# Rengar-Yang/humanoid-gym-with-comments

Measured on AMD Instinct MI355X. Metric: env-steps/sec (whole node) at 4096 envs + PPO iters/sec, 1/2/4/8 MI355X, higher is better.
Workload: dtype f32; 1 GPU; XBot-L flat terrain, 4096 envs/GPU, PPO 24-step rollout (BASELINE configs[1]); envs_per_gpu=4096, num_steps_per_env=24, parallelism=dp1, ppo=2 epochs x 4 minibatches, actor 705-512-256-128-12, critic 219-768-256-128-1, update_graph=one, gemm_table=tuning/tunableop_mi355x_f32.csv

## Files before the change

### humanoid-gym-with-comments_amd/csrc/hg_gemm.hip

```cpp
#include <hip/hip_runtime.h>
#include <stdint.h>

#include <type_traits>

#include "hg_common.h"

namespace {

typedef float f32x16 __attribute__((ext_vector_type(16)));
typedef float f32x4u __attribute__((ext_vector_type(4), aligned(4)));

struct GemmArgs {
  const float* A;
  int64_t lda;
  const float* B;
  int64_t ldb;
  const float* bias;
  const float* Y;
  int64_t ldY;
  float* C;
  int64_t ldc;
  float* colpart;
  int64_t M;
  int N, K;
// ... 906 lines not shown
  __device__ __forceinline__ void load(const float* __restrict__ P, int64_t ld, int64_t r0, int64_t rend, int col0,
                                       int ncols, int tid) {
#pragma unroll
    for (int j = 0; j < IPT; j++) {
      const int idx = tid + j * NT;
      if (ITEMS % NT != 0 && idx >= ITEMS) break;
      const int row = idx / (COLS / 4), c = col0 + 4 * (idx % (COLS / 4));
      const int64_t r = r0 + row;
      const float* p = P + r * ld + c;
      if (r < rend && c + 3 < ncols) {
        const f32x4u x = *reinterpret_cast<const f32x4u*>(p);
        v[j][0] = x[0]; v[j][1] = x[1]; v[j][2] = x[2]; v[j][3] = x[3];
      } else {
#pragma unroll
        for (int e = 0; e < 4; e++) v[j][e] = (r < rend && c + e < ncols) ? p[e] : 0.f;
      }
    }
  }
  __device__ __forceinline__ void store(char* __restrict__ S, int tid) const {
#pragma unroll
    for (int j = 0; j < IPT; j++) {
      const int idx = tid + j * NT;
      if (ITEMS % NT != 0 && idx >= ITEMS) break;
      const int row = idx / (COLS / 4), c4 = idx % (COLS / 4);
      uint2 x0, x1, x2;
      split3x4(v[j], x0, x1, x2);
      char* d = S + row * PITCH + 8 * c4;
      *reinterpret_cast<uint2*>(d) = x0;
      *reinterpret_cast<uint2*>(d + PLANE) = x1;
      *reinterpret_cast<uint2*>(d + 2 * PLANE) = x2;
    }
  }
};

template <int PITCH>
__device__ __forceinline__ bf16x8 tr_operand(const char* __restrict__ plane, int c0, int lane) {
  const int g = lane >> 4, q = (lane >> 2) & 3, p = lane & 3;
  const char* a = plane + (8 * (g >> 1) + q) * PITCH + 2 * (c0 + 16 * (g & 1) + 4 * p);
  typedef __attribute__((address_space(3))) s16x4 lds_s16x4;
  const s16x4 lo = __builtin_amdgcn_ds_read_tr16_b64_v4i16((lds_s16x4*)(a));
  const s16x4 hi = __builtin_amdgcn_ds_read_tr16_b64_v4i16((lds_s16x4*)(a + 4 * PITCH));
  const short e[8] = {lo[0], lo[1], lo[2], lo[3], hi[0], hi[1], hi[2], hi[3]};
  return __builtin_bit_cast(bf16x8, e);
}

template <int WGM, int WGN, int TM, int TN, int PF>
__global__ void __launch_bounds__(64 * WGM * WGN) k_wgrad_tr(WgradArgs w) {
  constexpr int NT = 64 * WGM * WGN;
  constexpr int BM = 32 * TM * WGM, BN = 32 * TN * WGN;
  typedef TrStage<BM, NT> SA;
  typedef TrStage<BN, NT> SB;
  constexpr int STAGE = 3 * SA::PLANE + 3 * SB::PLANE;
  __shared__ __attribute__((aligned(16))) char lds[2 * STAGE];
  const int tid = threadIdx.x, lane = tid & 63, wave = tid >> 6;
  const int i = lane & 31, h = lane >> 5;
  const unsigned nb = gridDim.x;
  unsigned L = blockIdx.x;
  if ((nb & 7u) == 0) L = (blockIdx.x & 7u) * (nb >> 3) + (blockIdx.x >> 3);
  if ((int64_t)L >= w.tiles * w.slices) return;
  const int slice = (int)((int64_t)L / w.tiles);
  const int64_t tile = (int64_t)L % w.tiles;
  const int m0 = (int)(tile / w.tiles_n) * BM, n0 = (int)(tile % w.tiles_n) * BN;
  const int wm0 = (wave % WGM) * (32 * TM), wn0 = (wave / WGM) * (32 * TN);
  const int64_t kbeg = (int64_t)slice * w.kslice;
  const int64_t kend = min<int64_t>(w.R, kbeg + w.kslice);
  const int nchunks = kend > kbeg ? (int)((kend - kbeg + 15) / 16) : 0;

  f32x16 acc[TM][TN];
#pragma unroll
  for (int m = 0; m < TM; m++)
#pragma unroll
    for (int n = 0; n < TN; n++) acc[m][n] = (f32x16)0.f;

  auto step = [&](int c, SA& la, SB& lb, const SA& ha, const SB& hb) {
    const char* cur = lds + (c & 1) * STAGE;
    char* nxt = lds + ((c + 1) & 1) * STAGE;
    if (c + PF < nchunks) {
      const int64_t r0 = kbeg + (int64_t)(c + PF) * 16;
      la.load(w.A, w.lda, r0, kend, m0, w.M, tid);
      lb.load(w.B, w.ldb, r0, kend, n0, w.N, tid);
    }
    bf16x8 a[3][TM], b[3][TN];
#pragma unroll
    for (int p = 0; p < 3; p++) {
#pragma unroll
      for (int m = 0; m < TM; m++) a[p][m] = tr_operand<SA::PITCH>(cur + p * SA::PLANE, wm0 + 32 * m, lane);
#pragma unroll
      for (int n = 0; n < TN; n++)
        b[p][n] = tr_operand<SB::PITCH>(cur + 3 * SA::PLANE + p * SB::PLANE, wn0 + 32 * n, lane);
    }
#pragma unroll
    for (int m = 0; m < TM; m++)
#pragma unroll
      for (int n = 0; n < TN; n++) {
        acc[m][n] = __builtin_amdgcn_mfma_f32_32x32x16_bf16(a[2][m], b[0][n], acc[m][n], 0, 0, 0);
        acc[m][n] = __builtin_amdgcn_mfma_f32_32x32x16_bf16(a[1][m], b[1][n], acc[m][n], 0, 0, 0);
        acc[m][n] = __builtin_amdgcn_mfma_f32_32x32x16_bf16(a[0][m], b[2][n], acc[m][n], 0, 0, 0);
        acc[m][n] = __builtin_amdgcn_mfma_f32_32x32x16_bf16(a[1][m], b[0][n], acc[m][n], 0, 0, 0);
        acc[m][n] = __builtin_amdgcn_mfma_f32_32x32x16_bf16(a[0][m], b[1][n], acc[m][n], 0, 0, 0);
        acc[m][n] = __builtin_amdgcn_mfma_f32_32x32x16_bf16(a[0][m], b[0][n], acc[m][n], 0, 0, 0);
      }
    if (c + 1 < nchunks) {
      ha.store(nxt, tid);
      hb.store(nxt + 3 * SA::PLANE, tid);
    }
    __syncthreads();
  };
  SA sa0, sa1;
  SB sb0, sb1;
  if (nchunks > 0) {
    sa0.load(w.A, w.lda, kbeg, kend, m0, w.M, tid);
    sb0.load(w.B, w.ldb, kbeg, kend, n0, w.N, tid);
    sa0.store(lds, tid);
    sb0.store(lds + 3 * SA::PLANE, tid);
    if (PF == 2 && nchunks > 1) {
      sa1.load(w.A, w.lda, kbeg + 16, kend, m0, w.M, tid);
      sb1.load(w.B, w.ldb, kbeg + 16, kend, n0, w.N, tid);
    }
  }
  __syncthreads();
  if (PF == 1) {
    for (int c = 0; c < nchunks; c++) step(c, sa0, sb0, sa0, sb0);
  } else {
    for (int c = 0; c < nchunks; c += 2) {
      step(c, sa0, sb0, sa1, sb1);
      if (c + 1 < nchunks) step(c + 1, sa1, sb1, sa0, sb0);
    }
  }
  float* Cs = w.C + (int64_t)slice * w.cstride;
#pragma unroll
  for (int n = 0; n < TN; n++) {
    const int col = n0 + wn0 + 32 * n + i;
    if (col >= w.N) continue;
#pragma unroll
    for (int m = 0; m < TM; m++)
#pragma unroll
      for (int q = 0; q < 16; q++) {
        const int row = m0 + wm0 + 32 * m + (q & 3) + 8 * (q >> 2) + 4 * h;
        if (row < w.M) Cs[(int64_t)row * w.ldc + col] = acc[m][n][q];
      }
  }
}

template <int WGM, int WGN, int TM, int TN, int PF = 1>
int launch_wgrad_tr(WgradArgs w, hipStream_t s) {
  constexpr int BM = 32 * TM * WGM, BN = 32 * TN * WGN;
  w.tiles_n = (w.N + BN - 1) / BN;
  w.tiles = (int64_t)((w.M + BM - 1) / BM) * w.tiles_n;
  if (w.tiles * w.slices > 0x7fffffff) return HG_ERR_ARG;
  hipLaunchKernelGGL((k_wgrad_tr<WGM, WGN, TM, TN, PF>), dim3((unsigned)(w.tiles * w.slices)), dim3(64 * WGM * WGN), 0, s, w);
  return hipGetLastError() == hipSuccess ? HG_OK : HG_ERR_HIP;
}

constexpr int WGRAD_TR0 = 40, WGRAD_TR1 = 54;

}

extern "C" int64_t hg_gemm_x6_image_bytes(int64_t rows, int64_t K) {
  if (rows <= 0 || K <= 0 || rows > 0x7fffffff || K > 0x7fffffff) return -1;
  return img_chunks(K) * 3 * img_rows(rows) * 2 * 16;
}

extern "C" int hg_gemm_x6_image_jobs_pitched(const float* const* P, const int64_t* ld, const int* trans,
                                             const int64_t* rows, const int64_t* K, void* const* img,
                                             const int64_t* pitch_rows, int njobs, void* stream);

extern "C" int hg_gemm_x6_image_jobs(const float* const* P, const int64_t* ld, const int* trans, const int64_t* rows,
                                     const int64_t* K, void* const* img, int njobs, void* stream) {
  return hg_gemm_x6_image_jobs_pitched(P, ld, trans, rows, K, img, nullptr, njobs, stream);
}

extern "C" int hg_gemm_x6_image_jobs_pitched(const float* const* P, const int64_t* ld, const int* trans,
                                             const int64_t* rows, const int64_t* K, void* const* img,
                                             const int64_t* pitch_rows, int njobs, void* stream) {
  if (njobs <= 0) return HG_OK;
  if (njobs > IMG_MAX || !P || !ld || !trans || !rows || !K || !img) return HG_ERR_ARG;
  ImageJobs J;
  J.njobs = njobs;
  int64_t blocks = 0;
  for (int j = 0; j < njobs; j++) {
    if (!P[j] || !img[j] || rows[j] <= 0 || K[j] <= 0 || rows[j] > 0x7fffffff || K[j] > 0x7fffffff ||
        (trans[j] != 0 && trans[j] != 1))
      return HG_ERR_ARG;
    if ((trans[j] == 0 && ld[j] < K[j]) || (trans[j] == 1 && ld[j] < rows[j])) return HG_ERR_ARG;
    if ((uintptr_t)P[j] % 4 || (uintptr_t)img[j] % 16) return HG_ERR_ARG;
    J.P[j] = P[j];
    J.img[j] = reinterpret_cast<bf16x8*>(img[j]);
    J.ld[j] = ld[j];
    const int64_t prow = pitch_rows && pitch_rows[j] > 0 ? pitch_rows[j] : rows[j];
    if (prow < rows[j] || prow > 0x7fffffff) return HG_ERR_ARG;
    J.pitch[j] = img_rows(prow) * 2;
    J.trans[j] = trans[j];
    J.R[j] = (int)rows[j];
    J.K[j] = (int)K[j];
    J.groups[j] = (int)(img_rows(rows[j]) / 128);
    J.block0[j] = (int)blocks;
    blocks += img_chunks(K[j]) * J.groups[j];
    if (blocks > (int64_t)1 << 30) return HG_ERR_ARG;
  }
  J.block0[njobs] = (int)blocks;
  for (int j = 0; j < njobs;) {
    const int64_t prow = pitch_rows && pitch_rows[j] > 0 ? pitch_rows[j] : rows[j];
    int64_t sum = rows[j];
    int e = j + 1;
    while (e < njobs && pitch_rows && pitch_rows[e] == prow && K[e] == K[j] && sum < prow &&
           (uintptr_t)img[e] == (uintptr_t)img[e - 1] + (uintptr_t)(32 * rows[e - 1])) {
      sum += rows[e];
      e++;
    }
    if (sum != prow) return HG_ERR_ARG;
    for (int b = j; b + 1 < e; b++)
      if (rows[b] % 256) return HG_ERR_ARG;
    j = e;
  }
  hipLaunchKernelGGL(k_x6_image_jobs, dim3((unsigned)blocks), dim3(256), 0, (hipStream_t)stream, J);
  return hipGetLastError() == hipSuccess ? HG_OK : HG_ERR_HIP;
}

extern "C" int hg_gemm_f32_img(int mode, const float* A, int64_t lda, const void* Aimg, const void* Bimg,
                               const float* bias, const float* Y, int64_t ldY, float* C, int64_t ldc, float* colpart,
                               int64_t M, int N, int K, int act, int tile, int64_t aimg_bytes, int64_t bimg_bytes,
                               void* stream) {
  if ((!A && !Aimg) || !Bimg || !C || M <= 0 || N <= 0 || K <= 0 || ldc < N || (mode != 0 && mode != 1) || act < 0 ||
      act > 1 || tile < 19 || tile > NTILES_IMG)
    return HG_ERR_ARG;
  if (!Aimg && lda < K) return HG_ERR_ARG;
  if (bimg_bytes != hg_gemm_x6_image_bytes(N, K) || (Aimg && aimg_bytes != hg_gemm_x6_image_bytes(M, K)))
    return HG_ERR_ARG;
  if (mode == 1 && act == 1 && (!Y || ldY < N)) return HG_ERR_ARG;
  if ((!Aimg && (uintptr_t)A % 4) || (uintptr_t)Aimg % 16 || (uintptr_t)Bimg % 16 || (uintptr_t)C % 4)
    return HG_ERR_ARG;
  const bool vec = !Aimg && lda % 4 == 0 && (uintptr_t)A % 16 == 0;
  const float* a = Aimg ? reinterpret_cast<const float*>(Aimg) : A;
  const int64_t la = Aimg ? img_rows(M) * 2 : lda;
  GemmArgs g{a, la, reinterpret_cast<const float*>(Bimg), img_rows(N) * 2, bias, Y, ldY, C, ldc, colpart, M, N, K, 0, 0};
  GemmX6Args xa{g, 0, 0, 1};
  return x6_img_dispatch(tile, mode, Aimg ? 3 : 1, xa, vec, act == 1, (hipStream_t)stream);
}

extern "C" int hg_gemm_f32_img_split(const float* A, int64_t lda, const void* Bimg, const float* bias,
                                     const float* bias2, float* C, int64_t ldc, float* C2, int64_t ldc2, int nsplit,
                                     int64_t M, int N, int K, int act, int tile, int64_t bimg_bytes, void* stream) {
  if (!A || !Bimg || !C || !C2 || !bias != !bias2 || M <= 0 || N <= 0 || K <= 0 || nsplit <= 0 || nsplit >= N || nsplit % 256 ||
      ldc < nsplit || ldc2 < N - nsplit || lda < K || act < 0 || act > 1 || tile < 19 || tile > NTILES_IMG)
    return HG_ERR_ARG;
  if (bimg_bytes != hg_gemm_x6_image_bytes(N, K)) return HG_ERR_ARG;
  if ((uintptr_t)A % 4 || (uintptr_t)Bimg % 16 || (uintptr_t)C % 4 || (uintptr_t)C2 % 4) return HG_ERR_ARG;
  const bool vec = lda % 4 == 0 && (uintptr_t)A % 16 == 0;
  GemmArgs g{A, lda, reinterpret_cast<const float*>(Bimg), img_rows(N) * 2, bias, nullptr, 0, C, ldc, nullptr, M, N, K,
             0, 0, C2, ldc2, nsplit, bias2};
  GemmX6Args xa{g, 0, 0, 1};
  return x6_img_dispatch(tile, 0, 1, xa, vec, act == 1, (hipStream_t)stream);
}

extern "C" int hg_gemm_wgrad_img(const void* Aimg, const void* Bimg, float* C, int64_t ldc, int64_t cstride, int64_t M,
                                 int N, int64_t K, int slices, int tile, int64_t aimg_bytes, int64_t bimg_bytes,
                                 void* stream) {
  if (!Aimg || !Bimg || !C || M <= 0 || N <= 0 || K <= 0 || K > 0x7fffffff || ldc < N || slices < 1 || tile < 19 ||
      tile > NTILES)
    return HG_ERR_ARG;
  if (aimg_bytes != hg_gemm_x6_image_bytes(M, K) || bimg_bytes != hg_gemm_x6_image_bytes(N, K)) return HG_ERR_ARG;
  if (slices > 1 && cstride < M * (int64_t)ldc) return HG_ERR_ARG;
  if ((uintptr_t)Aimg % 16 || (uintptr_t)Bimg % 16 || (uintptr_t)C % 4) return HG_ERR_ARG;
  GemmArgs g{reinterpret_cast<const float*>(Aimg), img_rows(M) * 2, reinterpret_cast<const float*>(Bimg),
             img_rows(N) * 2, nullptr, nullptr, 0, C, ldc, nullptr, M, N, (int)K, 0, 0};
  const int64_t kslice = ((K + slices - 1) / slices + 31) & ~(int64_t)31;
  GemmX6Args xa{g, kslice, cstride, slices};
  return x6_img_dispatch(tile, 2, 3, xa, false, false, (hipStream_t)stream);
}

extern "C" int hg_gemm_tile(int mode, int64_t M, int N, int K) {
  (void)mode;
  (void)K;
  const int64_t t16 = ((M + 127) / 128) * ((N + 63) / 64);
  return t16 >= 768 ? 16 : 5;
}

extern "C" int64_t hg_gemm_colpart_rows(int64_t M, int tile) {
  if (tile < 1 || tile > NTILES_IMG) return -1;
  const int bm = tile_bm(tile);
  return (M + bm - 1) / bm;
}

extern "C" int hg_gemm_f32(int mode, const float* A, int64_t lda, const float* B, int64_t ldb, const float* bias,
                           const float* Y, int64_t ldY, float* C, int64_t ldc, float* colpart, int64_t M, int N, int K,
                           int act, int tile, void* stream) {
  if (tile == 30) tile = 25;
  else if (tile == 31) tile = 22;
  else if (tile == 32) tile = 21;
  if (!A || !B || !C || M <= 0 || N <= 0 || K <= 0 || lda < K || ldc < N || mode < 0 || mode > 3 || mode == 2 ||
      act < 0 || act > 1 || tile < 1 || tile > NTILES)
    return HG_ERR_ARG;
  if (mode == 3 && tile < 19) return HG_ERR_ARG;
  if ((mode == 0 || mode == 3) && ldb < K) return HG_ERR_ARG;
  if (mode == 1 && ldb < N) return HG_ERR_ARG;
  if ((mode == 1 || mode == 3) && act == 1 && (!Y || ldY < N)) return HG_ERR_ARG;
  if ((uintptr_t)A % 4 || (uintptr_t)B % 4 || (uintptr_t)C % 4) return HG_ERR_ARG;
  const bool vec = lda % 4 == 0 && (uintptr_t)A % 16 == 0 &&
                   (mode == 1 || (ldb % 4 == 0 && (uintptr_t)B % 16 == 0));
  GemmArgs g{A, lda, B, ldb, bias, Y, ldY, C, ldc, colpart, M, N, K, 0, 0};
  hipStream_t s = (hipStream_t)stream;
  const bool elu = act == 1;
  switch (tile) {
    case 1: return launch<128, 128, 2, 2, 32, 0>(mode, g, vec, elu, s);
    case 2: return launch<128, 64, 2, 2, 32, 0>(mode, g, vec, elu, s);
    case 3: return launch<64, 128, 2, 2, 32, 0>(mode, g, vec, elu, s);
    case 4: return launch<64, 64, 2, 2, 32, 0>(mode, g, vec, elu, s);
    case 5: return launch<64, 64, 2, 2, 32, 1>(mode, g, vec, elu, s);
    case 6: return launch<64, 64, 2, 2, 64, 0>(mode, g, vec, elu, s);
    case 7: return launch<64, 64, 2, 2, 64, 1>(mode, g, vec, elu, s);
    case 8: return launch<128, 64, 4, 2, 32, 1>(mode, g, vec, elu, s);
    case 9: return launch<128, 128, 2, 4, 32, 1>(mode, g, vec, elu, s);
    case 10: return launch<128, 64, 2, 2, 64, 1>(mode, g, vec, elu, s);
    case 11: return launch<64, 64, 2, 2, 16, 1>(mode, g, vec, elu, s);
    case 12: return launch<128, 128, 2, 4, 16, 1>(mode, g, vec, elu, s);
    case 13: return launch<128, 64, 4, 2, 16, 1>(mode, g, vec, elu, s);
    case 14: return launch<64, 128, 2, 2, 16, 1>(mode, g, vec, elu, s);
    case 15: return launch<64, 64, 2, 2, 32, 1, 1>(mode, g, vec, elu, s);
    case 16: return launch<128, 64, 4, 2, 32, 1, 1>(mode, g, vec, elu, s);
    case 17: return launch<128, 128, 2, 4, 32, 1, 1>(mode, g, vec, elu, s);
    case 18: return launch<64, 64, 2, 2, 16, 1, 1>(mode, g, vec, elu, s);
    default: break;
  }
  GemmX6Args xa{g, 0, 0, 1};
  switch (tile) {
    case 20: return launch_x6<128, 128, 2, 2, 1>(mode, xa, vec, elu, s);
    case 21: return launch_x6<128, 128, 2, 4, 1>(mode, xa, vec, elu, s);
    case 22: return launch_x6<128, 64, 2, 2, 1>(mode, xa, vec, elu, s);
    case 29:
    case 23: return launch_x6<64, 64, 2, 2, 1>(mode, xa, vec, elu, s);
    case 24: return launch_x6<128, 128, 2, 2, 2>(mode, xa, vec, elu, s);
    case 25: return launch_x6<256, 128, 4, 2, 1>(mode, xa, vec, elu, s);
    case 26: return launch_x6<128, 128, 2, 4, 2>(mode, xa, vec, elu, s);
    case 27: return launch_x6<128, 256, 2, 4, 1>(mode, xa, vec, elu, s);
    case 28: return launch_x6<64, 256, 2, 4, 1>(mode, xa, vec, elu, s);
    default: return launch_x6<64, 128, 2, 2, 1>(mode, xa, vec, elu, s);
  }
}

extern "C" int hg_gemm_f32_wgrad(const float* A, int64_t lda, const float* B, int64_t ldb, float* C, int64_t ldc,
                                 int64_t cstride, int64_t M, int N, int64_t K, int slices, int kmajor, int tile,
                                 void* stream) {
  const bool tr = tile >= WGRAD_TR0 && tile <= WGRAD_TR1;
  if (!A || !B || !C || M <= 0 || N <= 0 || K <= 0 || ldc < N || slices < 1 || (!tr && (tile < 19 || tile > 28)) ||
      K > 0x7fffffff || (kmajor != 0 && kmajor != 1) || (tr && (kmajor != 0 || M > 0x7fffffff)))
    return HG_ERR_ARG;
  if (kmajor == 0 && (lda < M || ldb < N)) return HG_ERR_ARG;
  if (kmajor == 1 && (lda < K || ldb < K)) return HG_ERR_ARG;
  if (slices > 1 && cstride < M * (int64_t)ldc) return HG_ERR_ARG;
  if ((uintptr_t)A % 4 || (uintptr_t)B % 4 || (uintptr_t)C % 4) return HG_ERR_ARG;
  const int64_t kslice = ((K + slices - 1) / slices + 15) & ~(int64_t)15;
  hipStream_t s = (hipStream_t)stream;
  if (tr) {
    WgradArgs w{A, lda, B, ldb, C, ldc, cstride, (int)M, N, K, kslice, slices, 0, 0};
    switch (tile) {
      case 40: return launch_wgrad_tr<4, 2, 2, 3>(w, s);
      case 41: return launch_wgrad_tr<4, 2, 2, 2>(w, s);
      case 42: return launch_wgrad_tr<2, 2, 2, 2>(w, s);
      case 43: return launch_wgrad_tr<2, 4, 2, 2>(w, s);
      case 44: return launch_wgrad_tr<2, 2, 2, 3>(w, s);
      case 45: return launch_wgrad_tr<4, 2, 1, 2>(w, s);
      case 46: return launch_wgrad_tr<2, 2, 1, 1>(w, s);
      case 47: return launch_wgrad_tr<2, 2, 1, 2>(w, s);
      case 48: return launch_wgrad_tr<2, 2, 2, 1>(w, s);
      case 49: return launch_wgrad_tr<4, 2, 2, 3, 2>(w, s);
      case 50: return launch_wgrad_tr<4, 2, 2, 2, 2>(w, s);
      case 51: return launch_wgrad_tr<2, 2, 2, 2, 2>(w, s);
      case 52: return launch_wgrad_tr<2, 2, 1, 1, 2>(w, s);
      case 53: return launch_wgrad_tr<2, 2, 1, 2, 2>(w, s);
      default: return launch_wgrad_tr<4, 2, 1, 2, 2>(w, s);
    }
  }
  GemmArgs g{A, lda, B, ldb, nullptr, nullptr, 0, C, ldc, nullptr, M, N, (int)K, 0, 0};
  GemmX6Args xa{g, kslice, cstride, slices};
  const int md = kmajor ? 4 : 2;
  const bool vec = kmajor && lda % 4 == 0 && ldb % 4 == 0 && (uintptr_t)A % 16 == 0 && (uintptr_t)B % 16 == 0;
  switch (tile) {
    case 20: return launch_x6<128, 128, 2, 2, 1>(md, xa, vec, false, s);
    case 21: return launch_x6<128, 128, 2, 4, 1>(md, xa, vec, false, s);
    case 22: return launch_x6<128, 64, 2, 2, 1>(md, xa, vec, false, s);
    case 23: return launch_x6<64, 64, 2, 2, 1>(md, xa, vec, false, s);
    case 24: return launch_x6<128, 128, 2, 2, 2>(md, xa, vec, false, s);
    case 25: return launch_x6<256, 128, 4, 2, 1>(md, xa, vec, false, s);
    case 26: return launch_x6<128, 128, 2, 4, 2>(md, xa, vec, false, s);
    case 27: return launch_x6<128, 256, 2, 4, 1>(md, xa, vec, false, s);
    case 28: return launch_x6<64, 256, 2, 4, 1>(md, xa, vec, false, s);
    default: return launch_x6<64, 128, 2, 2, 1>(md, xa, vec, false, s);
  }
}

namespace {
template <bool ELU, int SC>
__global__ void __launch_bounds__(256) k_splitk_finish(const float* __restrict__ ws, int64_t sstride,
                                                       const float* __restrict__ bias, float* __restrict__ C,
                                                       int64_t ldc, int64_t M, int N, int S, bool vec) {
  const int nq = (N + 3) >> 2;
  const int64_t t = (int64_t)blockIdx.x * 256 + threadIdx.x;
  if (t >= M * nq) return;
  const int64_t m = t / nq;
  const int n0 = (int)(t % nq) * 4;
  const float* p = ws + m * N + n0;
  float v[4];
  if (vec) {
    float4 a;
    if (SC > 0) {
      typedef float fin4 __attribute__((ext_vector_type(4)));
      fin4 x[SC > 0 ? SC : 1];
#pragma unroll
      for (int s = 0; s < SC; s++) x[s] = __builtin_nontemporal_load(reinterpret_cast<const fin4*>(p + s * sstride));
#pragma unroll
      for (int s = 1; s < SC; s++) { x[0].x += x[s].x; x[0].y += x[s].y; x[0].z += x[s].z; x[0].w += x[s].w; }
      a = make_float4(x[0].x, x[0].y, x[0].z, x[0].w);
    } else {
      a = *reinterpret_cast<const float4*>(p);
      for (int s = 1; s < S; s++) {
        const float4 b = *reinterpret_cast<const float4*>(p + s * sstride);
        a.x += b.x; a.y += b.y; a.z += b.z; a.w += b.w;
      }
    }
    const float4 bb = *reinterpret_cast<const float4*>(bias + n0);
    v[0] = a.x + bb.x; v[1] = a.y + bb.y; v[2] = a.z + bb.z; v[3] = a.w + bb.w;
#pragma unroll
    for (int q = 0; q < 4; q++)
      if (ELU) v[q] = v[q] > 0.f ? v[q] : expm1f(v[q]);
    *reinterpret_cast<float4*>(C + m * ldc + n0) = make_float4(v[0], v[1], v[2], v[3]);
  } else {
    for (int q = 0; q < 4 && n0 + q < N; q++) {
      float a = p[q];
      for (int s = 1; s < S; s++) a += p[q + s * sstride];
      float x = a + bias[n0 + q];
      if (ELU) x = x > 0.f ? x : expm1f(x);
      C[m * ldc + n0 + q] = x;
    }
  }
}

int splitk_finish(const float* ws, const float* bias, float* C, int64_t ldc, int64_t M, int N, int slices, bool elu,
                  hipStream_t s) {
  const int64_t threads = M * ((N + 3) / 4);
  const bool fvec = N % 4 == 0 && ldc % 4 == 0 && (uintptr_t)C % 16 == 0 && (uintptr_t)bias % 16 == 0;
  const dim3 grid((unsigned)((threads + 255) / 256)), block(256);
#define HG_FIN(E, SC) hipLaunchKernelGGL((k_splitk_finish<E, SC>), grid, block, 0, s, ws, M * (int64_t)N, bias, C, ldc, M, N, \
                                         slices, fvec)
  if (elu) {
    if (slices == 4) HG_FIN(true, 4);
    else if (slices == 2) HG_FIN(true, 2);
    else HG_FIN(true, 0);
  } else {
    if (slices == 4) HG_FIN(false, 4);
    else if (slices == 2) HG_FIN(false, 2);
    else HG_FIN(false, 0);
  }
#undef HG_FIN
  return hipGetLastError() == hipSuccess ? HG_OK : HG_ERR_HIP;
}
}

extern "C" int64_t hg_gemm_splitk_kslice(int K, int slices) {
  if (K <= 0 || slices < 1) return -1;
  return (((int64_t)K + slices - 1) / slices + 15) & ~(int64_t)15;
}

extern "C" int hg_gemm_f32_splitk(const float* A, int64_t lda, const float* B, int64_t ldb, const float* bias,
                                  float* C, int64_t ldc, float* ws, int64_t ws_floats, int64_t M, int N, int K,
                                  int act, int tile, int slices, void* stream) {
  if (!A || !B || !bias || !C || !ws || M <= 0 || N <= 0 || K <= 0 || lda < K || ldb < K || ldc < N ||
      act < 0 || act > 1 || tile < 20 || tile > 28 || slices < 2 || slices > 16)
    return HG_ERR_ARG;
  const int64_t kslice = hg_gemm_splitk_kslice(K, slices);
  if ((slices - 1) * kslice >= K) return HG_ERR_ARG;
  if (ws_floats < slices * M * (int64_t)N) return HG_ERR_ARG;
  if ((uintptr_t)A % 4 || (uintptr_t)B % 4 || (uintptr_t)C % 4 || (uintptr_t)bias % 4 || (uintptr_t)ws % 16)
    return HG_ERR_ARG;
  const int64_t threads = M * ((N + 3) / 4);
  if ((threads + 255) / 256 > 0x7fffffff) return HG_ERR_ARG;
  hipStream_t s = (hipStream_t)stream;
  GemmArgs g{A, lda, B, ldb, nullptr, nullptr, 0, ws, N, nullptr, M, N, K, 0, 0};
  GemmX6Args xa{g, kslice, M * (int64_t)N, slices};
  const bool vec = lda % 4 == 0 && ldb % 4 == 0 && (uintptr_t)A % 16 == 0 && (uintptr_t)B % 16 == 0;
  const bool elu = act == 1;
  const int md = 4;
  int rc;
  switch (tile) {
    case 20: rc = launch_x6<128, 128, 2, 2, 1>(md, xa, vec, elu, s); break;
    case 21: rc = launch_x6<128, 128, 2, 4, 1>(md, xa, vec, elu, s); break;
    case 22: rc = launch_x6<128, 64, 2, 2, 1>(md, xa, vec, elu, s); break;
    case 23: rc = launch_x6<64, 64, 2, 2, 1>(md, xa, vec, elu, s); break;
    case 24: rc = launch_x6<128, 128, 2, 2, 2>(md, xa, vec, elu, s); break;
    case 25: rc = launch_x6<256, 128, 4, 2, 1>(md, xa, vec, elu, s); break;
    case 26: rc = launch_x6<128, 128, 2, 4, 2>(md, xa, vec, elu, s); break;
    case 27: rc = launch_x6<128, 256, 2, 4, 1>(md, xa, vec, elu, s); break;
    default: rc = launch_x6<64, 256, 2, 4, 1>(md, xa, vec, elu, s); break;
  }
  if (rc != HG_OK) return rc;
  return splitk_finish(ws, bias, C, ldc, M, N, slices, elu, s);
}

extern "C" int hg_gemm_f32_splitk_img(const float* A, int64_t lda, const void* Bimg, int64_t bimg_bytes,
                                      const float* bias, float* C, int64_t ldc, float* ws, int64_t ws_floats,
                                      int64_t M, int N, int K, int act, int tile, int slices, void* stream) {
  if (!A || !Bimg || !bias || !C || !ws || M <= 0 || N <= 0 || K <= 0 || lda < K || ldc < N || act < 0 || act > 1 ||
      tile < 19 || tile > NTILES_IMG || tile == 24 || tile == 26 || tile == 29 || slices < 2 || slices > 16)
    return HG_ERR_ARG;
  if (bimg_bytes != hg_gemm_x6_image_bytes(N, K)) return HG_ERR_ARG;
  const int64_t kslice = hg_gemm_splitk_kslice(K, slices);
  if ((slices - 1) * kslice >= K) return HG_ERR_ARG;
  if (ws_floats < slices * M * (int64_t)N) return HG_ERR_ARG;
  if ((uintptr_t)A % 4 || (uintptr_t)Bimg % 16 || (uintptr_t)C % 4 || (uintptr_t)bias % 4 || (uintptr_t)ws % 16)
    return HG_ERR_ARG;
  if ((M * ((N + 3) / 4) + 255) / 256 > 0x7fffffff) return HG_ERR_ARG;
  hipStream_t s = (hipStream_t)stream;
  GemmArgs g{A, lda, reinterpret_cast<const float*>(Bimg), img_rows(N) * 2, nullptr, nullptr, 0, ws, N, nullptr, M, N,
             K, 0, 0};
  GemmX6Args xa{g, kslice, M * (int64_t)N, slices};
  const bool vec = lda % 4 == 0 && (uintptr_t)A % 16 == 0;
  const int rc = x6_img_dispatch(tile, 4, 1, xa, vec, false, s);
  if (rc != HG_OK) return rc;
  return splitk_finish(ws, bias, C, ldc, M, N, slices, act == 1, s);
}
```

### humanoid-gym-with-comments_amd/humanoid/algo/ppo/hg_mlp.py

```python
import contextlib
import ctypes
import os

import torch
import torch.nn as nn
import torch.nn.functional as F

from humanoid import _native as N


def fusable(net):
    mods = list(net)
    if not mods or not isinstance(mods[-1], nn.Linear):
        return False
    for i, m in enumerate(mods):
        want = nn.Linear if i % 2 == 0 else nn.ELU
        if not isinstance(m, want):
            return False
        if isinstance(m, nn.ELU) and (m.alpha != 1.0 or m.inplace):
            return False
        if isinstance(m, nn.Linear) and m.bias is None:
            return False
    return True


class _Reductions:

    def __init__(self):
        self.jobs = []

    def add(self, src, dst, width, parts):
        self.jobs.append((src, dst, int(width), int(parts)))

    def launch(self, dev):
        n = len(self.jobs)
        if n == 0:
            return
        vp = ctypes.c_void_p
        src = (vp * n)(*[j[0].data_ptr() for j in self.jobs])
        dst = (vp * n)(*[j[1].data_ptr() for j in self.jobs])
        width = (ctypes.c_int64 * n)(*[j[2] for j in self.jobs])
        parts = (ctypes.c_int * n)(*[j[3] for j in self.jobs])
        rc = N.lib().hg_colsum_jobs(src, dst, width, parts, n, _stream(dev))
        if rc != 0:
            raise RuntimeError(f"hg_colsum_jobs failed ({rc})")
        self.jobs = []


def _act_backward(gy, y, rows, width, gb, red=None):
    L = N.lib()
    scratch = torch.empty(int(L.hg_mlp_act_backward_scratch(rows, width)), dtype=torch.float32, device=gy.device)
    gh = torch.empty_like(gy) if y is not None else gy
    s = ctypes.c_void_p(torch.cuda.current_stream(gy.device).cuda_stream)
    rc = L.hg_mlp_act_backward(gy.data_ptr(), y.data_ptr() if y is not None else None,
                               gh.data_ptr() if y is not None else None, rows, width,
                               gb.data_ptr() if red is None else None, scratch.data_ptr(), s)
    if rc != 0:
        raise RuntimeError(f"hg_mlp_act_backward failed ({rc})")
    if red is not None:
        red.add(scratch, gb, width, scratch.numel() // width)
    return gh


def _stream(dev):
    return ctypes.c_void_p(torch.cuda.current_stream(dev).cuda_stream)


def _skinny_ok(h, W):
    n, k = W.shape
    return (bool(N.lib().hg_linear_skinny_supported(n, k)) and h.dim() == 2 and h.stride(1) == 1
            and h.stride(0) % 4 == 0 and h.data_ptr() % 16 == 0 and W.is_contiguous())


def _skinny_forward(h, W, b, out=None):
    rows, n = h.shape[0], W.shape[0]
    y = torch.empty(rows, n, dtype=torch.float32, device=h.device) if out is None else out
    if y.numel() != rows * n or not y.is_contiguous() or y.dtype != torch.float32:
        raise RuntimeError("skinny forward: out must be a contiguous float32 tensor of rows x n elements")
    rc = N.lib().hg_linear_skinny_forward(h.data_ptr(), h.stride(0), W.data_ptr(), b.data_ptr(), y.data_ptr(), rows,
                                          n, W.shape[1], _stream(h.device))
    if rc != 0:
        raise RuntimeError(f"hg_linear_skinny_forward failed ({rc})")
    return y


def _skinny_backward(g, h, W, need_dx, red=None):
    rows, (n, k) = g.shape[0], W.shape
    L = N.lib()
    wb = torch.empty(n * k + n, dtype=torch.float32, device=g.device)
    dx = torch.empty(rows, k, dtype=torch.float32, device=g.device) if need_dx else None
    scratch = torch.empty(int(L.hg_linear_skinny_backward_scratch(rows, n, k)), dtype=torch.float32, device=g.device)
    rc = L.hg_linear_skinny_backward(g.data_ptr(), h.data_ptr(), h.stride(0), W.data_ptr(),
                                     dx.data_ptr() if need_dx else None, wb.data_ptr() if red is None else None,
                                     rows, n, k, scratch.data_ptr(), _stream(g.device))
    if rc != 0:
        raise RuntimeError(f"hg_linear_skinny_backward failed ({rc})")
    if red is not None:
        red.add(scratch, wb, n * k + n, scratch.numel() // (n * k + n))
    return wb[: n * k].view(n, k), wb[n * k:], dx


def _skinny_backward_act(g, h, W, red):
    rows, (n, k) = g.shape[0], W.shape
    L = N.lib()
    wb = torch.empty(n * k + n, dtype=torch.float32, device=g.device)
    gh_prev = torch.empty(rows, k, dtype=torch.float32, device=g.device)
    parts = int(L.hg_linear_skinny_colpart_rows(rows))
    cp = torch.empty(parts, k, dtype=torch.float32, device=g.device)
    gb_prev = torch.empty(k, dtype=torch.float32, device=g.device)
    scratch = torch.empty(int(L.hg_linear_skinny_backward_scratch(rows, n, k)), dtype=torch.float32, device=g.device)
    rc = L.hg_linear_skinny_backward_act(g.data_ptr(), h.data_ptr(), h.stride(0), W.data_ptr(), gh_prev.data_ptr(),
                                         cp.data_ptr(), rows, n, k, scratch.data_ptr(), _stream(g.device))
    if rc != 0:
        raise RuntimeError(f"hg_linear_skinny_backward_act failed ({rc})")
    r = red if red is not None else _Reductions()
    r.add(scratch, wb, n * k + n, scratch.numel() // (n * k + n))
    r.add(cp, gb_prev, k, parts)
    if red is None:
        r.launch(g.device)
    return wb[: n * k].view(n, k), wb[n * k:], gh_prev, gb_prev


_BIG_ROWS = 1 << 40
_DW_SPLIT = {(128, 256): 32, (128, 128): 16, (256, 512): 4, (128, 705): 8, (512, 705): 16, (768, 219): 32,
             (256, 768): 4}


WGRAD_TR = os.environ.get("HG_WGRAD_TR", "1") != "0"
_GEMM_DW = {(512, 705): [(8191, 0), (_BIG_ROWS, (49, 32))],
            (256, 768): [(8191, 0), (_BIG_ROWS, (49, 64))]} if WGRAD_TR else {}
if WGRAD_TR:
    _GEMM_DW[(768, 780)] = [(8191, 0), (_BIG_ROWS, (49, 32))]
_GEMM_DW_EXTRA = {(256, 512): (54, 64), (768, 219): (54, 64), (128, 705): (48, 64), (128, 256): (54, 128),
                  (128, 128): (46, 128)}
_sel = os.environ.get("HG_WGRAD_TR", "1")
if _sel not in ("0", "1"):
    for _shape, _route_tr in _GEMM_DW_EXTRA.items():
        if _sel == "all" or "%dx%d" % _shape in _sel.split(","):
            _GEMM_DW[_shape] = [(8191, 0), (_BIG_ROWS, _route_tr)]


def _weight_grad(gh, x, red=None):
    rows, n = gh.shape
    k = x.shape[1]
    ok = red is not None and gh.is_contiguous() and x.dim() == 2 and x.stride(1) == 1
    route = _route(_GEMM_DW, rows, n, k) if ok else 0
    if route:
        tile, S = route
        L = N.lib()
        part = torch.empty(S, n, k, dtype=torch.float32, device=gh.device)
        rc = L.hg_gemm_f32_wgrad(gh.data_ptr(), gh.stride(0), x.data_ptr(), x.stride(0), part.data_ptr(), k, n * k,
                                 n, k, rows, S, 0, tile, _stream(gh.device))
        if rc != 0:
            raise RuntimeError(f"hg_gemm_f32_wgrad failed ({rc})")
        dw = torch.empty(n, k, dtype=torch.float32, device=gh.device)
        red.add(part, dw, n * k, S)
        return dw
    S = _DW_SPLIT.get((n, k), 1) if rows >= 8192 else 1
    if S == 1 or rows % S or not (gh.is_contiguous() and x.is_contiguous()):
        return torch.mm(gh.t(), x)
    chunks = torch.bmm(gh.view(S, rows // S, n).transpose(1, 2), x.view(S, rows // S, k))
    if red is None:
        return chunks.sum(0)
    dw = torch.empty(n, k, dtype=torch.float32, device=gh.device)
    red.add(chunks, dw, n * k, S)
    return dw


_FUSED_FWD_ROWS = {(512, 256): 8192, (256, 128): 8192, (128, 128): 32768}
FUSED_FORWARD = os.environ.get("HG_FUSED_FORWARD", "1") != "0"


def _fused_ok(h, W, b):
    rows = h.shape[0]
    k = W.shape[1]
    return (FUSED_FORWARD and rows <= _FUSED_FWD_ROWS.get((k, W.shape[0]), 0) and h.dim() == 2 and h.stride(1) == 1
            and h.dtype == torch.float32 and W.is_contiguous() and b is not None and b.is_contiguous())


def linear_act(h, W, b, elu=True, out=None, tile=0):
    rows, n = h.shape[0], W.shape[0]
    y = torch.empty(rows, n, dtype=torch.float32, device=h.device) if out is None else out
    if y.shape != (rows, n) or y.stride(1) != 1 or y.dtype != torch.float32:
        raise RuntimeError("linear_act: out must be a float32 [rows, n] tensor with unit column stride")
    rc = N.lib().hg_linear_act_forward(h.data_ptr(), h.stride(0), W.data_ptr(), b.data_ptr(), y.data_ptr(),
                                       y.stride(0), rows, n, W.shape[1], 1 if elu else 0, tile, _stream(h.device))
    if rc != 0:
        raise RuntimeError(f"hg_linear_act_forward failed ({rc})")
    return y


_BIG = 1 << 40
X6_TILE0 = 19
_GEMM_FWD = {(705, 512): [(8192, 5), (_BIG, 20)], (512, 256): [(8192, 5), (_BIG, 22)],
             (256, 128): [(8192, 0), (32768, 5), (_BIG, 20)], (705, 128): [(8192, 5), (_BIG, 29)],
             (128, 128): [(8192, 0), (_BIG, 5)], (219, 768): [(8192, 21), (_BIG, 32)],
             (768, 256): [(32768, 22), (_BIG, 20)]}
if os.environ.get("HG_X6_APF", "1") == "0":
    _GEMM_FWD[(705, 128)] = [(8192, 5), (_BIG, 23)]
_GEMM_FWD[(780, 768)] = _GEMM_FWD[(219, 768)]
_GEMM_DX = {(256, 512): [(_BIG, 22)], (128, 256): [(_BIG, 31)], (256, 768): [(_BIG, 31)], (128, 128): [(_BIG, 5)]}
GEMM = os.environ.get("HG_GEMM", "1") != "0"
X6_IMAGE = os.environ.get("HG_X6_IMAGE", "1") != "0"
SKINNY_ACT = os.environ.get("HG_SKINNY_ACT", "1") != "0"


def _route(table, rows, k, n):
    if not GEMM:
        return 0
    for max_rows, tile in table.get((k, n), ()):
        if rows <= max_rows:
            return tile
    return 0


def _gemm_fwd_tile(h, W, b):
    if not (h.dim() == 2 and h.stride(1) == 1 and h.dtype == torch.float32 and W.is_contiguous() and b is not None
            and b.is_contiguous()):
        return 0
    return _route(_GEMM_FWD, h.shape[0], W.shape[1], W.shape[0])


_GEMM_FWD_SPLITK = {(705, 512): [(4096, (25, 4))]}
SPLITK_FWD = os.environ.get("HG_SPLITK_FWD", "1") != "0"
if os.environ.get("HG_SPLITK_ROUTE"):
    _GEMM_FWD_SPLITK[(705, 512)] = [(4096, tuple(int(v) for v in os.environ["HG_SPLITK_ROUTE"].split(",")))]


def _gemm_fwd_splitk(h, W, b):
    if not SPLITK_FWD or not _gemm_fwd_tile(h, W, b):
        return None
    for max_rows, route in _GEMM_FWD_SPLITK.get((W.shape[1], W.shape[0]), ()):
        if h.shape[0] <= max_rows:
            return route
    return None


def gemm_forward_splitk(h, W, b, tile, slices, elu=True):
    rows, n, k = h.shape[0], W.shape[0], W.shape[1]
    y = torch.empty(rows, n, dtype=torch.float32, device=h.device)
    ws = torch.empty(slices * rows * n, dtype=torch.float32, device=h.device)
    rc = N.lib().hg_gemm_f32_splitk(h.data_ptr(), h.stride(0), W.data_ptr(), W.stride(0), b.data_ptr(), y.data_ptr(),
                                    y.stride(0), ws.data_ptr(), ws.numel(), rows, n, k, 1 if elu else 0, tile, slices,
                                    _stream(h.device))
    if rc != 0:
        raise RuntimeError(f"hg_gemm_f32_splitk failed ({rc})")
    return y


def _img_rows(r):
    return (r + 255) // 256 * 256


def x6_images(jobs, dev):
    if not jobs:
        return []
    L = N.lib()

    def rows_of(j):
        return sum(P.shape[0] for P in j[1]) if j[0] == "stack" else j[2]

    sizes = [int(L.hg_gemm_x6_image_bytes(rows_of(j), j[-1])) for j in jobs]
    buf = torch.empty(sum(sizes) // 4, dtype=torch.float32, device=dev)
    imgs, off = [], 0
    for sz in sizes:
        imgs.append(buf[off // 4:(off + sz) // 4])
        off += sz
    cj = []
    for j, im in zip(jobs, imgs):
        if j[0] == "stack":
            total, r0 = rows_of(j), 0
            for P in j[1]:
                if r0 % 256:
                    raise ValueError("x6_images: stacked bands must start on a multiple of 256 rows "
                                     "(every band but the last a multiple of 256 rows)")
                cj.append((P, 0, P.shape[0], j[2], im.data_ptr() + 32 * r0, total))
                r0 += P.shape[0]
        else:
            cj.append((j[0], j[1], j[2], j[3], im.data_ptr(), 0))
    m = len(cj)
    vp = ctypes.c_void_p
    i64 = ctypes.c_int64
    rc = L.hg_gemm_x6_image_jobs_pitched((vp * m)(*[c[0].data_ptr() for c in cj]), (i64 * m)(*[c[0].stride(0) for c in cj]),
                                         (ctypes.c_int * m)(*[c[1] for c in cj]), (i64 * m)(*[c[2] for c in cj]),
                                         (i64 * m)(*[c[3] for c in cj]), (vp * m)(*[c[4] for c in cj]),
                                         (i64 * m)(*[c[5] for c in cj]), m, _stream(dev))
    if rc != 0:
        raise RuntimeError(f"hg_gemm_x6_image_jobs_pitched failed ({rc})")
    return imgs
# ... 533 lines not shown
```

Measured before the change: 5.885 million env-steps/s.

## Add software-pipelined transposed wgrad kernel with interleaved staging and MFMA scheduling

Adds a new weight-gradient kernel variant (tile 56) that double-buffers LDS stages and prefetches two chunks ahead in registers. It interleaves the bf16x3 split stores of the next stage between MFMA groups using sched_group_barrier, and adds an edge path that shifts partial-tile loads instead of masking them. It becomes the default route for the large 512x705, 256x768 and 768x780 wgrad shapes in place of tile 49. The goal is to hide global-load and LDS-staging latency behind the matrix math, at the cost of higher register pressure and more complex scheduling.

```diff
diff --git a/humanoid-gym-with-comments_amd/csrc/hg_gemm.hip b/humanoid-gym-with-comments_amd/csrc/hg_gemm.hip
--- a/humanoid-gym-with-comments_amd/csrc/hg_gemm.hip
+++ b/humanoid-gym-with-comments_amd/csrc/hg_gemm.hip
@@ -1082,7 +1082,337 @@
   return hipGetLastError() == hipSuccess ? HG_OK : HG_ERR_HIP;
 }
 
-constexpr int WGRAD_TR0 = 40, WGRAD_TR1 = 54;
+template <int COLS, int NT, int W>
+struct TrStageP {
+  static constexpr int CG = COLS / W;
+  static constexpr int TPR = NT / 16;
+  static_assert(NT % 16 == 0 && CG % TPR == 0 && (W == 2 || W == 4), "every thread carries CG / TPR items of its row");
+  static constexpr int IPT = CG / TPR;
+  static constexpr int PITCH = COLS * 2 + 64;
+  static constexpr int PLANE = 16 * PITCH;
+  typedef float vecu __attribute__((ext_vector_type(W), aligned(4)));
+  struct Map {
+    uint32_t goff;
+    int lds;
+    __device__ __forceinline__ void init(int64_t ld, int col0, int tid) {
+      const int row = tid / TPR, cg = tid % TPR;
+      goff = (uint32_t)(((int64_t)row * ld + col0 + W * cg) * 4);
+      lds = row * PITCH + 2 * W * cg;
+    }
+  };
+  struct EdgeMap {
+    uint32_t goff[IPT];
+    bool on[IPT][3];
+    __device__ __forceinline__ void init(int64_t ld, int col0, int ncols, int tid) {
+      const int row = tid / TPR;
+#pragma unroll
+      for (int j = 0; j < IPT; j++) {
+        const int c = col0 + W * (tid % TPR + j * TPR);
+        const int ce = max(0, min(c, ncols - W));
+        const int shift = min(c - ce, W);
+        goff[j] = (uint32_t)(((int64_t)row * ld + ce) * 4);
+#pragma unroll
+        for (int b = 0; b < 3; b++) on[j][b] = (shift >> b) & 1;
+      }
+    }
+  };
+  float v[IPT][W];
+  __device__ __forceinline__ void load(const float* __restrict__ P, int64_t ld, int64_t r0, int64_t rend, int col0,
+                                       int ncols, int tid, const Map& mp) {
+    const int64_t r = r0 + tid / TPR;
+    const char* base = reinterpret_cast<const char*>(P + r0 * ld);
+#pragma unroll
+    for (int j = 0; j < IPT; j++) {
+      const int c = col0 + W * (tid % TPR + j * TPR);
+      const float* p = reinterpret_cast<const float*>(base + mp.goff + 4 * W * TPR * j);
+      if (r < rend && c + W - 1 < ncols) {
+        const vecu x = *reinterpret_cast<const vecu*>(p);
+#pragma unroll
+        for (int e = 0; e < W; e++) v[j][e] = x[e];
+      } else {
+#pragma unroll
+        for (int e = 0; e < W; e++) v[j][e] = (r < rend && c + e < ncols) ? p[e] : 0.f;
+      }
+    }
+  }
+  __device__ __forceinline__ void load_full(const char* __restrict__ base, const Map& mp) {
+#pragma unroll
+    for (int j = 0; j < IPT; j++) {
+      const vecu x = *reinterpret_cast<const vecu*>(base + mp.goff + 4 * W * TPR * j);
+#pragma unroll
+      for (int e = 0; e < W; e++) v[j][e] = x[e];
+    }
+  }
+  __device__ __forceinline__ void load_full(const char* __restrict__ base, const EdgeMap& mp) {
+#pragma unroll
+    for (int j = 0; j < IPT; j++) {
+      const vecu x = *reinterpret_cast<const vecu*>(base + mp.goff[j]);
+#pragma unroll
+      for (int e = 0; e < W; e++) v[j][e] = x[e];
+    }
+  }
+  template <int j>
+  __device__ __forceinline__ void place_item(const Map&) {}
+  template <int j>
+  __device__ __forceinline__ void place_item(const EdgeMap& mp) {
+    float y[W];
+#pragma unroll
+    for (int e = 0; e < W; e++) {
+      y[e] = v[j][e];
+      asm("" : "+v"(y[e]));
+    }
+#pragma unroll
+    for (int b = 0; (1 << b) <= W; b++) {
+#pragma unroll
+      for (int e = 0; e < W; e++) y[e] = mp.on[j][b] ? (e + (1 << b) < W ? y[e + (1 << b) < W ? e + (1 << b) : e] : 0.f) : y[e];
+    }
+#pragma unroll
+    for (int e = 0; e < W; e++) v[j][e] = y[e];
+  }
+  __device__ __forceinline__ void store(char* __restrict__ S, const Map& mp) const {
+#pragma unroll
+    for (int j = 0; j < IPT; j++) store_one(S, mp, j);
+  }
+  template <int j>
+  __device__ __forceinline__ void store_item(char* __restrict__ S, const Map& mp) const {
+    store_one(S, mp, j);
+  }
+  __device__ __forceinline__ void store_one(char* __restrict__ S, const Map& mp, const int j) const {
+    {
+      char* d = S + mp.lds + 2 * W * TPR * j;
+      if (W == 4) {
+        uint2 x0, x1, x2;
+        split3x4(v[j], x0, x1, x2);
+        *reinterpret_cast<uint2*>(d) = x0;
+        *reinterpret_cast<uint2*>(d + PLANE) = x1;
+        *reinterpret_cast<uint2*>(d + 2 * PLANE) = x2;
+      } else {
+        f32x2 a = {v[j][0], v[j][1]};
+        const uint32_t a0 = bf16_pair(a);
+        a -= bf16_pair_f32(a0);
+        const uint32_t a1 = bf16_pair(a);
+        a -= bf16_pair_f32(a1);
+        *reinterpret_cast<uint32_t*>(d) = a0;
+        *reinterpret_cast<uint32_t*>(d + PLANE) = a1;
+        *reinterpret_cast<uint32_t*>(d + 2 * PLANE) = bf16_pair(a);
+      }
+    }
+  }
+};
+
+template <int N, int I = 0, class F>
+__device__ __forceinline__ void static_for(F&& f) {
+  if constexpr (I < N) {
+    f(std::integral_constant<int, I>());
+    static_for<N, I + 1>(f);
+  }
+}
+
+template <int PITCH>
+__device__ __forceinline__ bf16x8 tr_operand2(const char* __restrict__ plane, int c0, int lane) {
+  const int g = lane >> 4, q = (lane >> 2) & 3, p = lane & 3;
+  const char* a = plane + (8 * (g >> 1) + q) * PITCH + 2 * (c0 + 16 * (g & 1) + 4 * p);
+  typedef __attribute__((address_space(3))) s16x4 lds_s16x4;
+  const s16x4 lo = __builtin_amdgcn_ds_read_tr16_b64_v4i16((lds_s16x4*)(a));
+  const s16x4 hi = __builtin_amdgcn_ds_read_tr16_b64_v4i16((lds_s16x4*)(a + 4 * PITCH));
+  return __builtin_bit_cast(bf16x8, __builtin_shufflevector(lo, hi, 0, 1, 2, 3, 4, 5, 6, 7));
+}
+
+template <int WGM, int WGN, int TM, int TN>
+__global__ void __launch_bounds__(64 * WGM * WGN) k_wgrad_tr_pipe(WgradArgs w) {
+  constexpr int NT = 64 * WGM * WGN;
+  constexpr int BM = 32 * TM * WGM, BN = 32 * TN * WGN;
+  constexpr int WA = (BM / 4) % (NT / 16) == 0 ? 4 : 2, WB = (BN / 4) % (NT / 16) == 0 ? 4 : 2;
+  typedef TrStageP<BM, NT, WA> SA;
+  typedef TrStageP<BN, NT, WB> SB;
+  constexpr int STAGE = 3 * SA::PLANE + 3 * SB::PLANE;
+  __shared__ __attribute__((aligned(16))) char lds[2 * STAGE];
+  const int tid = threadIdx.x, lane = tid & 63;
+  const int wave = __builtin_amdgcn_readfirstlane(tid >> 6);
+  const int i = lane & 31, h = lane >> 5;
+  const unsigned nb = gridDim.x;
+  unsigned L = blockIdx.x;
+  if ((nb & 7u) == 0) L = (blockIdx.x & 7u) * (nb >> 3) + (blockIdx.x >> 3);
+  if ((int64_t)L >= w.tiles * w.slices) return;
+  const int slice = (int)((int64_t)L / w.tiles);
+  const int64_t tile = (int64_t)L % w.tiles;
+  const int m0 = (int)(tile / w.tiles_n) * BM, n0 = (int)(tile % w.tiles_n) * BN;
+  const int wm0 = (wave % WGM) * (32 * TM), wn0 = (wave / WGM) * (32 * TN);
+  const int64_t kbeg = (int64_t)slice * w.kslice;
+  const int64_t kend = min<int64_t>(w.R, kbeg + w.kslice);
+  const int nchunks = kend > kbeg ? (int)((kend - kbeg + 15) / 16) : 0;
+  const int nfull = kend > kbeg ? (int)((kend - kbeg) / 16) : 0;
+  const bool interior = m0 + BM <= w.M && n0 + BN <= w.N;
+  const bool shiftable = w.M >= WA && w.N >= WB;
+
+  f32x16 acc[TM][TN];
+#pragma unroll
+  for (int m = 0; m < TM; m++)
+#pragma unroll
+    for (int n = 0; n < TN; n++) acc[m][n] = (f32x16)0.f;
+
+  typename SA::Map ma;
+  typename SB::Map mb;
+  ma.init(w.lda, m0, tid);
+  mb.init(w.ldb, n0, tid);
+
+  auto mfma6 = [&](f32x16& c, const bf16x8 (&a)[3], const bf16x8 (&b)[3]) {
+    c = __builtin_amdgcn_mfma_f32_32x32x16_bf16(a[2], b[0], c, 0, 0, 0);
+    c = __builtin_amdgcn_mfma_f32_32x32x16_bf16(a[1], b[1], c, 0, 0, 0);
+    c = __builtin_amdgcn_mfma_f32_32x32x16_bf16(a[0], b[2], c, 0, 0, 0);
+    c = __builtin_amdgcn_mfma_f32_32x32x16_bf16(a[1], b[0], c, 0, 0, 0);
+    c = __builtin_amdgcn_mfma_f32_32x32x16_bf16(a[0], b[1], c, 0, 0, 0);
+    c = __builtin_amdgcn_mfma_f32_32x32x16_bf16(a[0], b[0], c, 0, 0, 0);
+  };
+  auto mfmas = [&](const char* cur) {
+    bf16x8 a[TM][3], b[TN][3];
+#pragma unroll
+    for (int m = 0; m < TM; m++)
+#pragma unroll
+      for (int p = 0; p < 3; p++) a[m][p] = tr_operand2<SA::PITCH>(cur + p * SA::PLANE, wm0 + 32 * m, lane);
+#pragma unroll
+    for (int n = 0; n < TN; n++)
+#pragma unroll
+      for (int p = 0; p < 3; p++)
+        b[n][p] = tr_operand2<SB::PITCH>(cur + 3 * SA::PLANE + p * SB::PLANE, wn0 + 32 * n, lane);
+#pragma unroll
+    for (int n = 0; n < TN; n++)
+#pragma unroll
+      for (int m = 0; m < TM; m++) mfma6(acc[m][n], a[m], b[n]);
+  };
+  auto step = [&](int c, SA& la, SB& lb, const SA& ha, const SB& hb) {
+    if (c + 2 < nchunks) {
+      const int64_t r0 = kbeg + (int64_t)(c + 2) * 16;
+      la.load(w.A, w.lda, r0, kend, m0, w.M, tid, ma);
+      lb.load(w.B, w.ldb, r0, kend, n0, w.N, tid, mb);
+    }
+    mfmas(lds + (c & 1) * STAGE);
+    if (c + 1 < nchunks) {
+      char* nxt = lds + ((c + 1) & 1) * STAGE;
+      ha.store(nxt, ma);
+      hb.store(nxt + 3 * SA::PLANE, mb);
+    }
+    __syncthreads();
+  };
+  constexpr int NI = SA::IPT + SB::IPT;
+  static_assert(NI <= TM * TN, "one staged item per slot");
+  auto fast = [&](const auto& ga, const auto& gb, int STG, const char* pa, const char* pb, SA& la, SB& lb, SA& ha,
+                  SB& hb) __attribute__((always_inline)) {
+    const char* cur = lds + STG * STAGE;
+    char* nxt = lds + (STG ^ 1) * STAGE;
+    la.load_full(pa, ga);
+    lb.load_full(pb, gb);
+    bf16x8 a[TM][3], b[TN][3];
+    auto read_a = [&](int m) {
+#pragma unroll
+      for (int p = 0; p < 3; p++) a[m][p] = tr_operand2<SA::PITCH>(cur + p * SA::PLANE, wm0 + 32 * m, lane);
+    };
+    auto read_b = [&](int n) {
+#pragma unroll
+      for (int p = 0; p < 3; p++)
+        b[n][p] = tr_operand2<SB::PITCH>(cur + 3 * SA::PLANE + p * SB::PLANE, wn0 + 32 * n, lane);
+    };
+    read_a(0);
+    read_b(0);
+    static_for<TM * TN>([&](auto SLOT) __attribute__((always_inline)) {
+      constexpr int slot = decltype(SLOT)::value, n = slot / TM, m = slot % TM;
+      constexpr bool reads = (n == 0 && m + 1 < TM) || (m == TM - 1 && n + 1 < TN);
+      __builtin_amdgcn_sched_barrier(0);
+      if constexpr (n == 0 && m + 1 < TM) read_a(m + 1);
+      if constexpr (m == TM - 1 && n + 1 < TN) read_b(n + 1);
+      if constexpr (slot < SA::IPT) {
+        ha.template place_item<slot>(ga);
+        ha.template store_item<slot>(nxt, ma);
+      } else if constexpr (slot < NI) {
+        hb.template place_item<slot - SA::IPT>(gb);
+        hb.template store_item<slot - SA::IPT>(nxt + 3 * SA::PLANE, mb);
+      }
+      mfma6(acc[m][n], a[m], b[n]);
+#pragma unroll
+      for (int k = 0; k < 6; k++) {
+        __builtin_amdgcn_sched_group_barrier(0x008, 1, 0);
+        if (reads) __builtin_amdgcn_sched_group_barrier(0x100, 1, 0);
+        if (slot < SA::IPT) __builtin_amdgcn_sched_group_barrier(0x002, 5, 0);
+        else if (slot < NI) __builtin_amdgcn_sched_group_barrier(0x002, 3, 0);
+      }
+    });
+    __builtin_amdgcn_sched_barrier(0);
+    __syncthreads();
+  };
+
+  SA sa0, sa1;
+  SB sb0, sb1;
+  const bool edge_loop = !interior && shiftable && nfull > 3;
+  typename SA::EdgeMap ea;
+  typename SB::EdgeMap eb;
+  if (nchunks > 0) {
+    sa0.load(w.A, w.lda, kbeg, kend, m0, w.M, tid, ma);
+    sb0.load(w.B, w.ldb, kbeg, kend, n0, w.N, tid, mb);
+    sa0.store(lds, ma);
+    sb0.store(lds + 3 * SA::PLANE, mb);
+    if (edge_loop) {
+      ea.init(w.lda, m0, w.M, tid);
+      eb.init(w.ldb, n0, w.N, tid);
+      sa1.load_full(reinterpret_cast<const char*>(w.A + (kbeg + 16) * w.lda), ea);
+      sb1.load_full(reinterpret_cast<const char*>(w.B + (kbeg + 16) * w.ldb), eb);
+    } else if (nchunks > 1) {
+      sa1.load(w.A, w.lda, kbeg + 16, kend, m0, w.M, tid, ma);
+      sb1.load(w.B, w.ldb, kbeg + 16, kend, n0, w.N, tid, mb);
+    }
+  }
+  __syncthreads();
+  int c = 0;
+  if (interior || edge_loop) {
+    const char* pa = reinterpret_cast<const char*>(w.A + (kbeg + 32) * w.lda);
+    const char* pb = reinterpret_cast<const char*>(w.B + (kbeg + 32) * w.ldb);
+    const int64_t sa16 = w.lda * 64, sb16 = w.ldb * 64;
+    auto pairs = [&](const auto& ga, const auto& gb) __attribute__((always_inline)) {
+      for (; c + 3 < nfull; c += 2) {
+        fast(ga, gb, 0, pa, pb, sa0, sb0, sa1, sb1);
+        fast(ga, gb, 1, pa + sa16, pb + sb16, sa1, sb1, sa0, sb0);
+        pa += 2 * sa16;
+        pb += 2 * sb16;
+      }
+    };
+    if (interior) {
+      pairs(ma, mb);
+    } else {
+      pairs(ea, eb);
+      static_for<SA::IPT>([&](auto J) __attribute__((always_inline)) { sa1.template place_item<decltype(J)::value>(ea); });
+      static_for<SB::IPT>([&](auto J) __attribute__((always_inline)) { sb1.template place_item<decltype(J)::value>(eb); });
+    }
+  }
+  for (; c < nchunks; c += 2) {
+    step(c, sa0, sb0, sa1, sb1);
+    if (c + 1 < nchunks) step(c + 1, sa1, sb1, sa0, sb0);
+  }
+  float* Cs = w.C + (int64_t)slice * w.cstride;
+#pragma unroll
+  for (int n = 0; n < TN; n++) {
+    const int col = n0 + wn0 + 32 * n + i;
+    if (col >= w.N) continue;
+#pragma unroll
+    for (int m = 0; m < TM; m++)
+#pragma unroll
+      for (int q = 0; q < 16; q++) {
+        const int row = m0 + wm0 + 32 * m + (q & 3) + 8 * (q >> 2) + 4 * h;
+        if (row < w.M) Cs[(int64_t)row * w.ldc + col] = acc[m][n][q];
+      }
+  }
+}
+
+template <int WGM, int WGN, int TM, int TN>
+int launch_wgrad_tr_pipe(WgradArgs w, hipStream_t s) {
+  constexpr int BM = 32 * TM * WGM, BN = 32 * TN * WGN;
+  if (w.lda >= (1 << 24) || w.ldb >= (1 << 24)) return HG_ERR_ARG;
+  w.tiles_n = (w.N + BN - 1) / BN;
+  w.tiles = (int64_t)((w.M + BM - 1) / BM) * w.tiles_n;
+  if (w.tiles * w.slices > 0x7fffffff) return HG_ERR_ARG;
+  hipLaunchKernelGGL((k_wgrad_tr_pipe<WGM, WGN, TM, TN>), dim3((unsigned)(w.tiles * w.slices)), dim3(64 * WGM * WGN), 0, s, w);
+  return hipGetLastError() == hipSuccess ? HG_OK : HG_ERR_HIP;
+}
+
+constexpr int WGRAD_TR0 = 40, WGRAD_TR1 = 54, WGRAD_TR_PIPE = 56;
 
 }
 
@@ -1271,7 +1601,7 @@
 extern "C" int hg_gemm_f32_wgrad(const float* A, int64_t lda, const float* B, int64_t ldb, float* C, int64_t ldc,
                                  int64_t cstride, int64_t M, int N, int64_t K, int slices, int kmajor, int tile,
                                  void* stream) {
-  const bool tr = tile >= WGRAD_TR0 && tile <= WGRAD_TR1;
+  const bool tr = (tile >= WGRAD_TR0 && tile <= WGRAD_TR1) || tile == WGRAD_TR_PIPE;
   if (!A || !B || !C || M <= 0 || N <= 0 || K <= 0 || ldc < N || slices < 1 || (!tr && (tile < 19 || tile > 28)) ||
       K > 0x7fffffff || (kmajor != 0 && kmajor != 1) || (tr && (kmajor != 0 || M > 0x7fffffff)))
     return HG_ERR_ARG;
@@ -1298,7 +1628,8 @@
       case 51: return launch_wgrad_tr<2, 2, 2, 2, 2>(w, s);
       case 52: return launch_wgrad_tr<2, 2, 1, 1, 2>(w, s);
       case 53: return launch_wgrad_tr<2, 2, 1, 2, 2>(w, s);
-      default: return launch_wgrad_tr<4, 2, 1, 2, 2>(w, s);
+      case 54: return launch_wgrad_tr<4, 2, 1, 2, 2>(w, s);
+      default: return launch_wgrad_tr_pipe<4, 2, 2, 3>(w, s);
     }
   }
   GemmArgs g{A, lda, B, ldb, nullptr, nullptr, 0, C, ldc, nullptr, M, N, (int)K, 0, 0};
diff --git a/humanoid-gym-with-comments_amd/humanoid/algo/ppo/hg_mlp.py b/humanoid-gym-with-comments_amd/humanoid/algo/ppo/hg_mlp.py
--- a/humanoid-gym-with-comments_amd/humanoid/algo/ppo/hg_mlp.py
+++ b/humanoid-gym-with-comments_amd/humanoid/algo/ppo/hg_mlp.py
@@ -127,14 +127,15 @@
 
 
 WGRAD_TR = os.environ.get("HG_WGRAD_TR", "1") != "0"
-_GEMM_DW = {(512, 705): [(8191, 0), (_BIG_ROWS, (49, 32))],
-            (256, 768): [(8191, 0), (_BIG_ROWS, (49, 64))]} if WGRAD_TR else {}
+_TR_TILE = 49 if os.environ.get("HG_WGRAD_TR") == "49" else 56
+_GEMM_DW = {(512, 705): [(8191, 0), (_BIG_ROWS, (_TR_TILE, 32))],
+            (256, 768): [(8191, 0), (_BIG_ROWS, (_TR_TILE, 64))]} if WGRAD_TR else {}
 if WGRAD_TR:
-    _GEMM_DW[(768, 780)] = [(8191, 0), (_BIG_ROWS, (49, 32))]
+    _GEMM_DW[(768, 780)] = [(8191, 0), (_BIG_ROWS, (_TR_TILE, 32))]
 _GEMM_DW_EXTRA = {(256, 512): (54, 64), (768, 219): (54, 64), (128, 705): (48, 64), (128, 256): (54, 128),
                   (128, 128): (46, 128)}
 _sel = os.environ.get("HG_WGRAD_TR", "1")
-if _sel not in ("0", "1"):
+if _sel not in ("0", "1", "49"):
     for _shape, _route_tr in _GEMM_DW_EXTRA.items():
         if _sel == "all" or "%dx%d" % _shape in _sel.split(","):
             _GEMM_DW[_shape] = [(8191, 0), (_BIG_ROWS, _route_tr)]
```

Measured after the change: 5.923 million env-steps/s, median of 6. Within noise of the previous version (+0.7%).
